# leabouffaut/DAS4Whales

Measured on AMD Instinct MI355X. Metric: channel-samples/sec through f-k filter + matched-filter, higher is better.
Workload: dtype f32 (matched filter: 2 x f16 split operands on the matrix cores, f32 accumulate); 1 GPU; 20000 channels x 120000 samples float32 per GPU, classic f-k fan mask (fk_filter_design defaults), stages fk+mf, HF+LF fin-call templates; api=public, parallelism=independent channel blocks x1

## Files before the change

das4whales_amd/csrc/mm_common.h:

```cpp
#pragma once
#include "fft_radix.h"

namespace d4w {

constexpr float kMmLoScale = 2048.f, kMmLoInv = 1.0f / 2048.f;

#ifdef D4W_EMU
typedef uint16_t mm_half;
struct alignas(16) mm_h8 { uint16_t v[8]; };
struct mm_f4 { float v[4]; };
__device__ __forceinline__ mm_half mm_to_half(float x) { return hipemu::f32_to_f16(x); }
__device__ __forceinline__ float mm_to_float(mm_half h) { return hipemu::f16_to_f32(h); }
__device__ __forceinline__ mm_f4 mm_zero() { return mm_f4{{0.f, 0.f, 0.f, 0.f}}; }
__device__ __forceinline__ mm_f4 mm_mfma(const mm_h8& a, const mm_h8& b, mm_f4 c) {
    hipemu::mfma_f32_16x16x32_f16(a.v, b.v, c.v);
    return c;
}
__device__ __forceinline__ float mm_get(const mm_f4& c, int r) { return c.v[r]; }
__device__ __forceinline__ void mm_set(mm_h8& a, int j, mm_half h) { a.v[j] = h; }
__device__ __forceinline__ int mm_uniform(int v) { return v; }
__device__ __forceinline__ void mm_sched_fence() {}
__device__ __forceinline__ void mm_store4(float* p, float a, float b, float c, float d) { p[0] = a; p[1] = b; p[2] = c; p[3] = d; }
__device__ __forceinline__ void mm_store1(float* p, float v) { *p = v; }
__device__ __forceinline__ float4 mm_load4_stream(const float4* p) { return *p; }
__device__ __forceinline__ void mm_put4(mm_half* p, const mm_half (&h)[4]) { p[0] = h[0]; p[1] = h[1]; p[2] = h[2]; p[3] = h[3]; }
__device__ __forceinline__ float mm_sqrt(float v) { return sqrtf(v); }
__device__ __forceinline__ void mm_wave_sync() { (void)__shfl_xor(0, 1); }
__device__ __forceinline__ float mm_clamp_half(float v) { return fminf(fmaxf(v, -65504.f), 65504.f); }
static inline int mm_num_cus() { return 2; }
#else
typedef _Float16 mm_half;
typedef _Float16 mm_h8 __attribute__((ext_vector_type(8)));
typedef _Float16 mm_h4 __attribute__((ext_vector_type(4)));
typedef float mm_f4 __attribute__((ext_vector_type(4)));
__device__ __forceinline__ mm_half mm_to_half(float x) { return (_Float16)x; }
__device__ __forceinline__ float mm_to_float(mm_half h) { return (float)h; }
__device__ __forceinline__ mm_f4 mm_zero() { mm_f4 z = {0.f, 0.f, 0.f, 0.f}; return z; }
__device__ __forceinline__ mm_f4 mm_mfma(mm_h8 a, mm_h8 b, mm_f4 c) { return __builtin_amdgcn_mfma_f32_16x16x32_f16(a, b, c, 0, 0, 0); }
__device__ __forceinline__ float mm_get(const mm_f4& c, int r) { return c[r]; }
__device__ __forceinline__ void mm_set(mm_h8& a, int j, mm_half h) { a[j] = h; }
__device__ __forceinline__ int mm_uniform(int v) { return __builtin_amdgcn_readfirstlane(v); }
__device__ __forceinline__ void mm_sched_fence() { __builtin_amdgcn_sched_barrier(0); }
__device__ __forceinline__ void mm_store4(float* p, float a, float b, float c, float d) {
    mm_f4 t = {a, b, c, d};
    __builtin_nontemporal_store(t, reinterpret_cast<mm_f4*>(p));
}
__device__ __forceinline__ void mm_store1(float* p, float v) { __builtin_nontemporal_store(v, p); }
__device__ __forceinline__ float4 mm_load4_stream(const float4* p) {
    const mm_f4 v = __builtin_nontemporal_load(reinterpret_cast<const mm_f4*>(p));
    return make_float4(v.x, v.y, v.z, v.w);
}
__device__ __forceinline__ void mm_put4(mm_half* p, const mm_half (&h)[4]) {
    mm_h4 v = {h[0], h[1], h[2], h[3]};
    *reinterpret_cast<mm_h4*>(p) = v;
}
__device__ __forceinline__ float mm_sqrt(float v) { return __builtin_amdgcn_sqrtf(v); }
// ... 74 lines not shown
```

das4whales_amd/csrc/xcorr_mm.hip:

```cpp
#include <cstdlib>

#include "mm_common.h"

namespace d4w {

#ifndef D4W_MM_CH
#define D4W_MM_CH 4096
#endif
constexpr int kMmCH = D4W_MM_CH;
constexpr int kMmKS = 6;
constexpr int kMmKSLong = 8;
constexpr int kMmKSMax = 16;
constexpr int kMmSection = 32 * kMmKSMax - 16;
constexpr int kMmMaxSupport = 32 * kMmKSLong - 15;
constexpr int kMmMaxSections = 16;
constexpr int kMmThreads = 256;
template <int KSM>
struct MmGeom {
    static constexpr int Halo = 32 * KSM;
    static constexpr int Stage = kMmCH + Halo;
    static constexpr int Q = (Stage + 4 * kMmThreads - 1) / (4 * kMmThreads);
    static constexpr int LastQ = (Stage - (Q - 1) * 4 * kMmThreads) / 4;
    static constexpr int Arr = Stage + 8;
};
__host__ __device__ constexpr int mm_pidx(int h) { return h; }

struct MmArgs {
    const float* x;
    const float* xnext;
    const double* mean;
    const float* maxabs;
    const float* taps;
    float* y0;
    float* y1;
    int nx, ns, ld_next, n_next, ltaps, len0, len1;
    float* rowmax0;
    float* rowmax1;
    int clamp;
// ... 12 lines not shown
    return v;
#else
    auto dpp = [](float x, auto ctrl, auto rmask) {
        return __int_as_float(__builtin_amdgcn_update_dpp(0, __float_as_int(x), decltype(ctrl)::value, decltype(rmask)::value, 0xf, false));
    };
    v += dpp(v, std::integral_constant<int, 0x111>{}, std::integral_constant<int, 0xf>{});
    v += dpp(v, std::integral_constant<int, 0x112>{}, std::integral_constant<int, 0xf>{});
    v += dpp(v, std::integral_constant<int, 0x114>{}, std::integral_constant<int, 0xf>{});
    v += dpp(v, std::integral_constant<int, 0x118>{}, std::integral_constant<int, 0xf>{});
    v += dpp(v, std::integral_constant<int, 0x142>{}, std::integral_constant<int, 0xa>{});
    v += dpp(v, std::integral_constant<int, 0x143>{}, std::integral_constant<int, 0xc>{});
    return v;
#endif
}

template <int KS0, int KS1, int WPS, bool TAIL = false, bool WMAX = false, bool WSPLIT = false>
__global__ __launch_bounds__(kMmThreads, WPS) void xcorr_mm_rows(MmArgs P) {
    static_assert(!(WSPLIT && KS1 > 0), "the wave-split kernel is the one-template code run by two wave pairs");
    constexpr int KSM = KS0 > KS1 ? KS0 : KS1;
    using GEO = MmGeom<KSM>;
    constexpr int kMmHalo = GEO::Halo, kMmStage = GEO::Stage, kMmQ = GEO::Q, kMmLastQ = GEO::LastQ, kMmArr = GEO::Arr;
    constexpr int kSeg = 4 * kMmQ;
    D4W_DYN_LDS(smem_raw);
    mm_half* lds = reinterpret_cast<mm_half*>(smem_raw);
    float* red = reinterpret_cast<float*>(lds + 4 * kMmArr);
    constexpr int kBlk = kMmCH / 4;
    float* pb = red + 8;
    float* wt = pb + 2 * kBlk;
    const int tid = (int)threadIdx.x;
    const int lane = tid & 63, wv = mm_uniform(tid >> 6);
    const int n16 = lane & 15, g = lane >> 4;
    const int ns = P.ns;
    const int tsel = WSPLIT ? (wv >> 1) : 0;

    const int nchunk = (ns + kMmCH - 1) / kMmCH;
    const long long total = (long long)P.nx * nchunk;
    const int nparts = min(8, (int)gridDim.x);
    const int xcd = (int)blockIdx.x % nparts, wq = (int)blockIdx.x / nparts, nq = ((int)gridDim.x - xcd + nparts - 1) / nparts;
    const long long lo_c = total * xcd / nparts, hi_c = total * (xcd + 1) / nparts;
    mm_h8 a0h[KS0], a0l[KS0];
    mm_h8 a1h[KS1 ? KS1 : 1], a1l[KS1 ? KS1 : 1];
    float osc0 = 1.f, osc1 = 1.f;
#ifdef D4W_MM_V_TAIL_DEALT
    constexpr bool kRows = false;
#else
    constexpr bool kRows = TAIL;
#endif
    auto next_chunk = [&](long long c) -> long long {
        if constexpr (kRows) {
            const long long r = c / nchunk;
            return (c - r * nchunk + 1 < nchunk) ? c + 1 : (r + (long long)gridDim.x) * nchunk;
        } else {
            return c + nq;
        }
    };
    const long long end_c = kRows ? total : hi_c;
    long long c_n = kRows ? (long long)blockIdx.x * nchunk : lo_c + wq;
    {
        float* tl = reinterpret_cast<float*>(smem_raw);
        constexpr int TLP = 16 + kMmHalo;
        for (int i = tid; i < 2 * TLP; i += kMmThreads) {
            const int t = i / TLP, u = i - t * TLP - 15;
            const int L = t ? P.len1 : P.len0;
            float tv = (u >= 0 && u < L && (t == 0 || KS1 > 0 || WSPLIT)) ? P.taps[(size_t)t * P.ltaps + u] : 0.f;
            if constexpr (TAIL) {
                if (u < L && (t == 0 || KS1 > 0 || WSPLIT)) tv += t ? P.tail1 : P.tail0;
            }
            tl[i] = tv;
        }
        __syncthreads();
        auto build = [&](const float* tp, int L, auto& ah, auto& al, auto ks, float& osc) {
            constexpr int KS = decltype(ks)::value;
// ... 14 lines not shown
                    mm_set(ah[kk], j, hi);
                    mm_set(al[kk], j, lo);
                });
            });
        };
        build(tl + (WSPLIT ? tsel * TLP : 0), WSPLIT && tsel ? P.len1 : P.len0, a0h, a0l, std::integral_constant<int, KS0>{}, osc0);
        if constexpr (KS1 > 0) build(tl + TLP, P.len1, a1h, a1l, std::integral_constant<int, KS1>{}, osc1);
        __syncthreads();
    }

    float4 pre[kMmQ];
    Mean2 mu_n{0.f, 0.f};
    float g_n = 1.f;
    bool heavy_n = false;
    bool tail_n = false;
    int row_n = 0, c0_n = 0;

    auto issue = [&](long long c) {
        row_n = (int)(c / nchunk);
        c0_n = (int)(c - (long long)row_n * nchunk) * kMmCH;
        mu_n = mean2_load(P.mean, row_n);
        g_n = 1.f;
        const int s0 = c0_n + P.shift;
        tail_n = s0 + kMmStage > ns;
        if (P.maxabs) {
            const float a = P.maxabs[row_n];
            g_n = (a > 0.f) ? 1.0f / a : 0.f;
            heavy_n = fabsf(mu_n.hi) > 0.9921875f * a;
        }
        const float* xr = P.x + (size_t)row_n * ns;
        const bool al = (reinterpret_cast<uintptr_t>(xr + s0) & 15) == 0;
        if (al && s0 + kMmStage <= ns) {
            const float4* p = reinterpret_cast<const float4*>(xr + s0) + tid;
            static_for<kMmQ>([&](auto qq) {
                constexpr int q = decltype(qq)::value;
                if (q < kMmQ - 1 || tid < kMmLastQ) pre[q] = mm_load4_stream(p + q * kMmThreads);
            });
        } else {
            if (al && (ns & 3) == 0) {
                static_for<kMmQ>([&](auto qq) {
                    constexpr int q = decltype(qq)::value;
                    if (q < kMmQ - 1 || tid < kMmLastQ) {
                        const int i = s0 + 4 * (tid + q * kMmThreads);
                        const float4 v = *reinterpret_cast<const float4*>(xr + min(i, ns - 4));
                        pre[q] = (i < ns) ? v : make_float4(mu_n.hi, mu_n.hi, mu_n.hi, mu_n.hi);
// ... 16 lines not shown
                    constexpr int q = decltype(qq)::value;
                    if (q < kMmQ - 1 || tid < kMmLastQ) {
                        const int d = s0 + 4 * (tid + q * kMmThreads) - ns;
                        const float b0 = xn[min(max(d, 0), n_next - 1)], b1 = xn[min(max(d + 1, 0), n_next - 1)];
                        const float b2 = xn[min(max(d + 2, 0), n_next - 1)], b3 = xn[min(max(d + 3, 0), n_next - 1)];
                        if (d >= 0 && d < n_next) pre[q].x = b0;
                        if (d + 1 >= 0 && d + 1 < n_next) pre[q].y = b1;
                        if (d + 2 >= 0 && d + 2 < n_next) pre[q].z = b2;
                        if (d + 3 >= 0 && d + 3 < n_next) pre[q].w = b3;
                    }
                });
            }
        }
    };

    if (c_n < end_c) issue(c_n);
    int buf = 0;
    constexpr bool want_max = WMAX;
    float pst_hi = 0.f, pst_lo = 0.f;
    for (long long c = c_n; c < end_c;) {
        const int row = row_n, c0 = c0_n;
        const Mean2 mu = mu_n;
        const bool tail = tail_n;
        const int n_valid = ns + ((P.xnext && P.n_next > 0) ? P.n_next : 0) - c0 - P.shift;
        float gsc = g_n, osx = 1.f;
        const float gout = g_n;
        const bool own_scale = !P.maxabs || heavy_n;
        mm_half* bh = lds + (size_t)buf * 2 * kMmArr;
        mm_half* bl = bh + kMmArr;
        const long long c_next = next_chunk(c);
        const int cin = c0 / kMmCH;
        if (TAIL && cin == 0) { pst_hi = 0.f; pst_lo = 0.f; }
        const float pst = pst_hi;
        if (own_scale) {
            float m = 0.f;
            static_for<kMmQ>([&](auto qq) {
                constexpr int q = decltype(qq)::value;
                if (q < kMmQ - 1 || tid < kMmLastQ) {
                    const float4 v = pre[q];
                    const int at = 4 * (tid + q * kMmThreads);
                    float d0 = demean(v.x, mu), d1 = demean(v.y, mu), d2 = demean(v.z, mu), d3 = demean(v.w, mu);
                    if (tail) {
                        if (at >= n_valid) d0 = 0.f;
                        if (at + 1 >= n_valid) d1 = 0.f;
                        if (at + 2 >= n_valid) d2 = 0.f;
                        if (at + 3 >= n_valid) d3 = 0.f;
                    }
                    m = fmaxf(fmaxf(m, fmaxf(fabsf(d0), fabsf(d1))), fmaxf(fabsf(d2), fabsf(d3)));
                }
            });
            for (int o = 32; o > 0; o >>= 1) m = fmaxf(m, __shfl_xor(m, o));
            if (lane == 0) red[wv + 4 * buf] = m;
            lds_barrier();
            m = fmaxf(fmaxf(red[4 * buf], red[4 * buf + 1]), fmaxf(red[4 * buf + 2], red[4 * buf + 3]));
            mm_pow2_scale(m, osx, gsc);
        }
        const float mlg = -mu.lo * gsc;
        static_for<kMmQ>([&](auto qq) {
            constexpr int q = decltype(qq)::value;
            float s[4] = {0.f, 0.f, 0.f, 0.f};
            const bool mine = q < kMmQ - 1 || tid < kMmLastQ;
            const int at = mm_pidx(4 * (tid + q * kMmThreads));
            if (mine) {
                const float4 v = pre[q];
#ifdef D4W_MM_V_FLOATMEAN
                s[0] = (v.x - mu.hi) * gsc; s[1] = (v.y - mu.hi) * gsc; s[2] = (v.z - mu.hi) * gsc; s[3] = (v.w - mu.hi) * gsc;
#else
                s[0] = fmaf(v.x - mu.hi, gsc, mlg); s[1] = fmaf(v.y - mu.hi, gsc, mlg); s[2] = fmaf(v.z - mu.hi, gsc, mlg); s[3] = fmaf(v.w - mu.hi, gsc, mlg);
#endif
                if (P.clamp && !own_scale) static_for<4>([&](auto ee) { constexpr int e = decltype(ee)::value; s[e] = mm_clamp_half(s[e]); });
                if (tail) {
                    const int a0 = 4 * (tid + q * kMmThreads);
                    static_for<4>([&](auto ee) { constexpr int e = decltype(ee)::value; if (a0 + e >= n_valid) s[e] = 0.f; });
                }
#ifdef D4W_MM_V_OLDSPLIT
                mm_half h[4], l[4];
                static_for<4>([&](auto ee) { constexpr int e = decltype(ee)::value; mm_split(s[e], h[e], l[e]); });
                mm_put4(bh + at, h);
                mm_put4(bl + at, l);
#else
                mm_split_put4(s, bh + at, bl + at);
#endif
            }
#ifdef D4W_MM_V_TAIL_NOSCAN
            if constexpr (false) {
#else
            if constexpr (TAIL && q < kMmCH / (4 * kMmThreads)) {
#endif
                const float t4 = (s[0] + s[1]) + (s[2] + s[3]);
                const float inc = mm_wave_scan(t4);
                pb[buf * kBlk + kMmThreads * q + tid] = inc - t4;
                if (lane == 63) wt[buf * 16 + 4 * q + wv] = inc;
            }
        });
        if (c_next < end_c) issue(c_next);
        lds_barrier();
        float* ya = ((WSPLIT && tsel) ? P.y1 : P.y0) + (size_t)row * ns;
        float* yb = KS1 ? P.y1 + (size_t)row * ns : nullptr;
        const bool valign = ((reinterpret_cast<uintptr_t>(ya + c0) & 15) == 0) && (!KS1 || (reinterpret_cast<uintptr_t>(yb + c0) & 15) == 0);
        const float oxs = (own_scale && P.maxabs) ? osx * gout : osx;
        const float o0 = osc0 * oxs, o1 = osc1 * oxs;
        float segoff = 0.f;
        constexpr int NTW = kMmCH / 256 / (WSPLIT ? 2 : 4), NST = NTW * KSM, PF = 2;
        auto tile_of = [&](int ti) { return WSPLIT ? (wv & 1) + 2 * ti : wv + 4 * ti; };
        auto frag = [&](const mm_half* arr, int T, int kk) -> mm_h8 {
            const int gr = 32 * T + 2 * n16 + g + 4 * kk;
            return *reinterpret_cast<const mm_h8*>(arr + mm_pidx(8 * gr));
        };
        mm_h8 fh[PF + 1], fl[PF + 1];
        static_for<PF>([&](auto ss) {
            constexpr int s_ = decltype(ss)::value;
            fh[s_] = frag(bh, tile_of(s_ / KSM), s_ % KSM);
            fl[s_] = frag(bl, tile_of(s_ / KSM), s_ % KSM);
        });
        mm_f4 c0h = mm_zero(), c0l = mm_zero(), c1h = mm_zero(), c1l = mm_zero();
        float vmax0 = -INFINITY, vmax1 = -INFINITY;
        float vsum = 0.f;
        static_for<NST>([&](auto ss) {
            constexpr int s_ = decltype(ss)::value, ti = s_ / KSM, kk = s_ % KSM;
            if constexpr (s_ + PF < NST) {
                fh[(s_ + PF) % (PF + 1)] = frag(bh, tile_of((s_ + PF) / KSM), (s_ + PF) % KSM);
                fl[(s_ + PF) % (PF + 1)] = frag(bl, tile_of((s_ + PF) / KSM), (s_ + PF) % KSM);
            }
            mm_sched_fence();
            const mm_h8 xh = fh[s_ % (PF + 1)], xl = fl[s_ % (PF + 1)];
            if constexpr (kk < KS0) {
                c0h = mm_mfma(a0h[kk], xh, c0h);
                c0l = mm_mfma(a0h[kk], xl, c0l);
            }
            if constexpr (kk < KS1) {
                c1h = mm_mfma(a1h[kk], xh, c1h);
                c1l = mm_mfma(a1h[kk], xl, c1l);
            }
            if constexpr (kk < KS0) c0l = mm_mfma(a0l[kk], xh, c0l);
            if constexpr (kk < KS1) c1l = mm_mfma(a1l[kk], xh, c1l);
            mm_sched_fence();
            if constexpr (kk == KSM - 1) {
                const int T = tile_of(ti);
                const int kl = 256 * T + 16 * n16 + 4 * g;
                const int k = c0 + kl;
                if constexpr (ti == 0) {
                if constexpr (TAIL) {
                    const float w = lane < 16 ? wt[buf * 16 + lane] : 0.f;
                    const float inc = mm_wave_scan(w);
                    segoff = inc - w;
        #ifdef D4W_EMU
                    const float own = __shfl(inc, 15);
        #else
                    const float own = __builtin_bit_cast(float, __builtin_amdgcn_readlane(__builtin_bit_cast(int, inc), 15));
        #endif
                    const double pd = ((double)pst_hi + (double)pst_lo) + (double)(own * oxs);
                    const float ph = (float)pd, pl2 = (float)(pd - (double)ph);
        #ifdef D4W_EMU
                    pst_hi = ph; pst_lo = pl2;
        #else
                    pst_hi = __builtin_bit_cast(float, __builtin_amdgcn_readfirstlane(__builtin_bit_cast(int, ph)));
                    pst_lo = __builtin_bit_cast(float, __builtin_amdgcn_readfirstlane(__builtin_bit_cast(int, pl2)));
        #endif
                }
                }
                float r0[4], r1[4];
                float a0 = 0.f, a1 = 0.f;
#ifdef D4W_MM_V_TAIL_NOSCAN
                if constexpr (false) {
#else
                if constexpr (TAIL) {
#endif
#ifdef D4W_EMU
                    const float so = __shfl(segoff, T);
#else
                    const float so = __builtin_bit_cast(float, __builtin_amdgcn_readlane(__builtin_bit_cast(int, segoff), T));
#endif
                    const float pbk = fmaf(so + pb[buf * kBlk + kMmThreads * (T >> 2) + 64 * (T & 3) + 4 * n16], oxs, pst);
                    a0 = ((WSPLIT && tsel) ? P.tail1 : P.tail0) * pbk;
                    a1 = P.tail1 * pbk;
                }
                static_for<4>([&](auto rr) {
                    constexpr int r = decltype(rr)::value;
                    r0[r] = fmaf(fmaf(mm_get(c0l, r), kMmLoInv, mm_get(c0h, r)), o0, a0);
                    if constexpr (KS1 > 0) r1[r] = fmaf(fmaf(mm_get(c1l, r), kMmLoInv, mm_get(c1h, r)), o1, a1);
                });
                c0h = mm_zero(); c0l = mm_zero(); c1h = mm_zero(); c1l = mm_zero();
                if (valign && k + 3 < ns) {
                    if (KS1 == 0 && P.accumulate) {
                        const float4 o = mm_load4_stream(reinterpret_cast<const float4*>(ya + k));
                        r0[0] += o.x; r0[1] += o.y; r0[2] += o.z; r0[3] += o.w;
                    }
                    mm_store4(ya + k, r0[0], r0[1], r0[2], r0[3]);
                    if constexpr (KS1 > 0) mm_store4(yb + k, r1[0], r1[1], r1[2], r1[3]);
                    if (want_max) {
                        vmax0 = fmaxf(vmax0, fmaxf(fmaxf(r0[0], r0[1]), fmaxf(r0[2], r0[3])));
#ifndef D4W_MM_V_NONAN
                        vsum += (r0[0] + r0[1]) + (r0[2] + r0[3]);
#endif
                        if constexpr (KS1 > 0) {
                            vmax1 = fmaxf(vmax1, fmaxf(fmaxf(r1[0], r1[1]), fmaxf(r1[2], r1[3])));
#ifndef D4W_MM_V_NONAN
// ... 16 lines not shown
                }
            }
        });
        if (want_max) {
            for (int o = 32; o > 0; o >>= 1) {
                vmax0 = fmaxf(vmax0, __shfl_xor(vmax0, o));
                if constexpr (KS1 > 0) vmax1 = fmaxf(vmax1, __shfl_xor(vmax1, o));
            }
            const bool bad = __any(vsum != vsum);
            if (lane == 0) {
                mm_atomic_fmax(((WSPLIT && tsel) ? P.rowmax1 : P.rowmax0) + row, bad ? __uint_as_float(0x7FC00000u) : vmax0);
                if constexpr (KS1 > 0) mm_atomic_fmax(P.rowmax1 + row, bad ? __uint_as_float(0x7FC00000u) : vmax1);
            }
        }
        buf ^= 1;
        c = c_next;
    }
}

}

using namespace d4w;

extern "C" {

int d4w_xcorr_mm_max_support(void) { return kMmSection * kMmMaxSections; }

#define D4W_MM_LAUNCH(KS0, KS1, WPS, TAIL, grid, lds, stream, Q)                                                              \
    do {                                                                                                                      \
        if ((Q).rowmax0) D4W_LAUNCH((xcorr_mm_rows<KS0, KS1, WPS, TAIL, true>), dim3(grid), dim3(kMmThreads), lds, stream, Q);  \
        else D4W_LAUNCH((xcorr_mm_rows<KS0, KS1, WPS, TAIL, false>), dim3(grid), dim3(kMmThreads), lds, stream, Q);             \
    } while (0)

static int mm_one_template(MmArgs P, const float* taps, int len, float* y, float* rowmax, int grid, void* stream) {
    auto lds_of = [](int arr) { return (size_t)4 * arr * sizeof(mm_half) + 8 * sizeof(float); };
    const int nsec = (len <= 32 * kMmKSMax - 15) ? 1 : ceil_div(len, kMmSection);
    const int per = (nsec == 1) ? len : 16 * ceil_div(ceil_div(len, nsec), 16);
    for (int j = 0; j < nsec; ++j) {
        const int first = j * per;
        MmArgs Q = P;
        Q.taps = taps + first;
        Q.len0 = Q.len1 = std::min(per, len - first);
        Q.y0 = y;
        Q.y1 = nullptr;
        Q.shift = first;
        Q.accumulate = j > 0;
        Q.rowmax0 = (j == nsec - 1) ? rowmax : nullptr;
        Q.rowmax1 = nullptr;
        const int ks = ceil_div(Q.len0 + 15, 32);
        if (ks <= kMmKS)
            D4W_MM_LAUNCH(kMmKS, 0, 3, false, grid, lds_of(MmGeom<kMmKS>::Arr), stream, Q);
        else if (ks <= kMmKSLong)
            D4W_MM_LAUNCH(kMmKSLong, 0, 2, false, grid, lds_of(MmGeom<kMmKSLong>::Arr), stream, Q);
        else if (ks <= 12)
            D4W_MM_LAUNCH(12, 0, 2, false, grid, lds_of(MmGeom<12>::Arr), stream, Q);
        else
            D4W_MM_LAUNCH(kMmKSMax, 0, 2, false, grid, lds_of(MmGeom<kMmKSMax>::Arr), stream, Q);
    }
    return D4W_OK;
}

int d4w_xcorr_mm_f32(const float* x, int nx, int ns, const float* xnext, int ld_next, int n_next, const double* mean,
                     const float* maxabs, const float* taps, int ntpl, int ltaps, int len0, int len1, float* y0, float* y1,
                     void* stream) {
    return d4w_xcorr_mm_rowmax_f32(x, nx, ns, xnext, ld_next, n_next, mean, maxabs, taps, ntpl, ltaps, len0, len1, y0, y1, nullptr,
                                   nullptr, stream);
}

int d4w_xcorr_mm_rowmax_f32(const float* x, int nx, int ns, const float* xnext, int ld_next, int n_next, const double* mean,
                            const float* maxabs, const float* taps, int ntpl, int ltaps, int len0, int len1, float* y0, float* y1,
                            float* rowmax0, float* rowmax1, void* stream) {
    return d4w_xcorr_mm_tail_f32(x, nx, ns, xnext, ld_next, n_next, mean, maxabs, taps, ntpl, ltaps, len0, len1, 0.0, 0.0, y0, y1,
// ... 18 lines not shown
        if (std::max(len0, len1) > d4w_xcorr_mm_tail_max_support())
            return fail(D4W_EINVAL, "with a tail the supports (%d, %d) must be <= %d", len0, len1, d4w_xcorr_mm_tail_max_support());
    }
    MmArgs P;
    P.x = x; P.xnext = xnext; P.mean = mean; P.maxabs = maxabs; P.taps = taps; P.y0 = y0; P.y1 = y1;
    P.nx = nx; P.ns = ns; P.ld_next = ld_next; P.n_next = xnext ? n_next : 0; P.ltaps = ltaps; P.len0 = len0; P.len1 = len1;
    P.shift = 0; P.accumulate = 0;
    static const int env_clamp = [] { const char* v = getenv("D4W_MM_CLAMP"); return v ? atoi(v) : 0; }();
    P.clamp = (xnext != nullptr && n_next > 0) || env_clamp;
    P.rowmax0 = rowmax0; P.rowmax1 = (ntpl == 2) ? rowmax1 : nullptr;
    P.tail0 = (float)tail0; P.tail1 = (float)tail1;
    if (rowmax0) {
        D4W_HIP(hipMemsetD32Async((hipDeviceptr_t)rowmax0, (int)0xFF800000u, (size_t)nx, (hipStream_t)stream));
        if (ntpl == 2) D4W_HIP(hipMemsetD32Async((hipDeviceptr_t)rowmax1, (int)0xFF800000u, (size_t)nx, (hipStream_t)stream));
    }
    const int nchunk = ceil_div(ns, kMmCH);
    const long long total = (long long)nx * nchunk;
    static const int env_wgs = [] { const char* v = getenv("D4W_MM_WGS"); const int n = v ? atoi(v) : 0; return n < 0 ? 0 : (n > 8 ? 8 : n); }();
    const int ks0 = ceil_div(len0 + 15, 32), ks1 = ceil_div(len1 + 15, 32);
    const bool fused = ntpl == 2 && std::max(ks0, ks1) <= kMmKS;
    const int per_cu = env_wgs ? env_wgs : ((ntpl == 1 && ks0 <= kMmKS) ? 3 : 2);
    const int ncu = mm_num_cus();
    const int grid = (int)std::min<long long>(total, (long long)ncu * per_cu);
    auto lds_of = [](int arr, bool tl) {
        return (size_t)4 * arr * sizeof(mm_half) + 8 * sizeof(float) + (tl ? ((size_t)2 * (kMmCH / 4) + 2 * 16) * sizeof(float) : 0);
    };
    static const int fused_form = [] { const char* v = getenv("D4W_MM_FUSED"); return v ? atoi(v) : 2; }();
    const int per_cu_ws = env_wgs ? env_wgs : 3;
#define D4W_MM_LAUNCH_WS(TAIL, grid, lds, Q)                                                                                            \
    do {                                                                                                                                \
        if ((Q).rowmax0) D4W_LAUNCH((xcorr_mm_rows<kMmKS, 0, 3, TAIL, true, true>), dim3(grid), dim3(kMmThreads), lds, stream, Q);       \
        else D4W_LAUNCH((xcorr_mm_rows<kMmKS, 0, 3, TAIL, false, true>), dim3(grid), dim3(kMmThreads), lds, stream, Q);                  \
    } while (0)
    if (tails) {
        const int grid_t = (int)std::min<long long>((long long)nx, (long long)ncu * per_cu);
        if (fused && fused_form != 2) {
            D4W_MM_LAUNCH_WS(true, (int)std::min<long long>((long long)nx, (long long)ncu * per_cu_ws), lds_of(MmGeom<kMmKS>::Arr, true), P);
            return D4W_OK;
        }
        if (fused) {
            const size_t lds = lds_of(MmGeom<kMmKS>::Arr, true);
            if (ks0 <= 5)
                D4W_MM_LAUNCH(5, kMmKS, 2, true, grid_t, lds, stream, P);
            else
                D4W_MM_LAUNCH(kMmKS, kMmKS, 2, true, grid_t, lds, stream, P);
            return D4W_OK;
        }
        for (int t = 0; t < ntpl; ++t) {
            MmArgs Q = P;
            Q.taps = taps + (size_t)t * ltaps;
            Q.len0 = Q.len1 = t ? len1 : len0;
            Q.tail0 = t ? (float)tail1 : (float)tail0;
            Q.tail1 = 0.f;
            Q.y0 = t ? y1 : y0;
            Q.y1 = nullptr;
            Q.rowmax0 = t ? rowmax1 : rowmax0;
            Q.rowmax1 = nullptr;
            const int ks = ceil_div(Q.len0 + 15, 32);
            if (ks <= kMmKS) {
                if (Q.rowmax0)
                    D4W_LAUNCH((xcorr_mm_rows<kMmKS, 0, 2, true, true>), dim3(grid_t), dim3(kMmThreads), lds_of(MmGeom<kMmKS>::Arr, true), stream, Q);
                else
                    D4W_LAUNCH((xcorr_mm_rows<kMmKS, 0, 3, true, false>), dim3(grid_t), dim3(kMmThreads), lds_of(MmGeom<kMmKS>::Arr, true), stream, Q);
            }
            else if (ks <= kMmKSLong)
                D4W_MM_LAUNCH(kMmKSLong, 0, 2, true, grid_t, lds_of(MmGeom<kMmKSLong>::Arr, true), stream, Q);
            else if (ks <= 12)
                D4W_MM_LAUNCH(12, 0, 2, true, grid_t, lds_of(MmGeom<12>::Arr, true), stream, Q);
            else
                D4W_MM_LAUNCH(kMmKSMax, 0, 2, true, grid_t, lds_of(MmGeom<kMmKSMax>::Arr, true), stream, Q);
        }
        return D4W_OK;
    }
    if (!fused) {
        int rc = mm_one_template(P, taps, len0, y0, rowmax0, grid, stream);
        if (rc == D4W_OK && ntpl == 2) rc = mm_one_template(P, taps + ltaps, len1, y1, rowmax1, grid, stream);
        return rc;
    }
    const size_t lds = lds_of(MmGeom<kMmKS>::Arr, false);
    if (fused_form != 2) {
        D4W_MM_LAUNCH_WS(false, (int)std::min<long long>(total, (long long)ncu * per_cu_ws), lds, P);
        return D4W_OK;
    }
    if (ks0 <= 5)
        D4W_MM_LAUNCH(5, kMmKS, 2, false, grid, lds, stream, P);
    else
        D4W_MM_LAUNCH(kMmKS, kMmKS, 2, false, grid, lds, stream, P);
    return D4W_OK;
}

}
```

Baseline: 117.3 billion channel-samples/s.

## Process paired 8192-sample chunks as two halo groups in fused matched filter

The fused two-template matched-filter kernel now handles 8192-sample chunks, split internally into two 4096-sample groups. Each group has its own halo and its own power-of-two scale, so per-block overhead (mean and maxabs loads, barriers, issue logic) is amortized over twice the samples. Chunk iteration switches from a 64-bit divide per chunk to incremental row, chunk and offset counters, and the per-row mean and scale load is skipped for later chunks in row mode. The cost is a larger LDS footprint, which may need the dynamic shared memory attribute and may reduce occupancy, plus extra halo conversion work and more register pressure from the per-group arrays.

```diff
diff --git a/das4whales_amd/csrc/mm_common.h b/das4whales_amd/csrc/mm_common.h
--- a/das4whales_amd/csrc/mm_common.h
+++ b/das4whales_amd/csrc/mm_common.h
@@ -19,6 +19,7 @@
 __device__ __forceinline__ float mm_get(const mm_f4& c, int r) { return c.v[r]; }
 __device__ __forceinline__ void mm_set(mm_h8& a, int j, mm_half h) { a.v[j] = h; }
 __device__ __forceinline__ int mm_uniform(int v) { return v; }
+__device__ __forceinline__ float mm_uniform(float v) { return v; }
 __device__ __forceinline__ void mm_sched_fence() {}
 __device__ __forceinline__ void mm_store4(float* p, float a, float b, float c, float d) { p[0] = a; p[1] = b; p[2] = c; p[3] = d; }
 __device__ __forceinline__ void mm_store1(float* p, float v) { *p = v; }
@@ -40,6 +41,7 @@
 __device__ __forceinline__ float mm_get(const mm_f4& c, int r) { return c[r]; }
 __device__ __forceinline__ void mm_set(mm_h8& a, int j, mm_half h) { a[j] = h; }
 __device__ __forceinline__ int mm_uniform(int v) { return __builtin_amdgcn_readfirstlane(v); }
+__device__ __forceinline__ float mm_uniform(float v) { return __builtin_bit_cast(float, __builtin_amdgcn_readfirstlane(__builtin_bit_cast(int, v))); }
 __device__ __forceinline__ void mm_sched_fence() { __builtin_amdgcn_sched_barrier(0); }
 __device__ __forceinline__ void mm_store4(float* p, float a, float b, float c, float d) {
     mm_f4 t = {a, b, c, d};
diff --git a/das4whales_amd/csrc/xcorr_mm.hip b/das4whales_amd/csrc/xcorr_mm.hip
--- a/das4whales_amd/csrc/xcorr_mm.hip
+++ b/das4whales_amd/csrc/xcorr_mm.hip
@@ -8,6 +8,8 @@
 #define D4W_MM_CH 4096
 #endif
 constexpr int kMmCH = D4W_MM_CH;
+constexpr int kMmCHPair = 8192;
+constexpr int kMmGroup = 4096;
 constexpr int kMmKS = 6;
 constexpr int kMmKSLong = 8;
 constexpr int kMmKSMax = 16;
@@ -15,13 +17,23 @@
 constexpr int kMmMaxSupport = 32 * kMmKSLong - 15;
 constexpr int kMmMaxSections = 16;
 constexpr int kMmThreads = 256;
-template <int KSM>
+template <int KSM, int CH = kMmCH>
 struct MmGeom {
+    static constexpr int G = CH > kMmGroup ? CH / kMmGroup : 1;
+    static constexpr int GL = CH / G;
     static constexpr int Halo = 32 * KSM;
-    static constexpr int Stage = kMmCH + Halo;
+    static constexpr int Stage = CH + Halo;
     static constexpr int Q = (Stage + 4 * kMmThreads - 1) / (4 * kMmThreads);
     static constexpr int LastQ = (Stage - (Q - 1) * 4 * kMmThreads) / 4;
-    static constexpr int Arr = Stage + 8;
+    static constexpr int GStage = GL + Halo;
+    static constexpr int Arr = G * GStage + 8;
+    static constexpr int QG = GL / (4 * kMmThreads);
+    static constexpr int Blk = CH / 4;
+    static constexpr int Pb = G == 1 ? Blk : Blk / 4;
+    static constexpr size_t lds_bytes(bool tail) {
+        return (size_t)4 * Arr * sizeof(mm_half) + 8 * G * sizeof(float) + (tail ? ((size_t)2 * Pb + 2 * 16 * G) * sizeof(float) : 0);
+    }
+    static_assert(CH % (4 * kMmThreads) == 0 && GL % (4 * kMmThreads) == 0 && Halo <= 4 * kMmThreads, "a group is whole loads; its halo lies in one");
 };
 __host__ __device__ constexpr int mm_pidx(int h) { return h; }
 
@@ -64,30 +76,24 @@
 #endif
 }
 
-template <int KS0, int KS1, int WPS, bool TAIL = false, bool WMAX = false, bool WSPLIT = false>
+template <int KS0, int KS1, int WPS, bool TAIL = false, bool WMAX = false, bool WSPLIT = false, int CH = kMmCH>
 __global__ __launch_bounds__(kMmThreads, WPS) void xcorr_mm_rows(MmArgs P) {
     static_assert(!(WSPLIT && KS1 > 0), "the wave-split kernel is the one-template code run by two wave pairs");
     constexpr int KSM = KS0 > KS1 ? KS0 : KS1;
-    using GEO = MmGeom<KSM>;
+    using GEO = MmGeom<KSM, CH>;
     constexpr int kMmHalo = GEO::Halo, kMmStage = GEO::Stage, kMmQ = GEO::Q, kMmLastQ = GEO::LastQ, kMmArr = GEO::Arr;
-    constexpr int kSeg = 4 * kMmQ;
+    constexpr int G = GEO::G, GL = GEO::GL, QG = GEO::QG, kPb = GEO::Pb;
     D4W_DYN_LDS(smem_raw);
     mm_half* lds = reinterpret_cast<mm_half*>(smem_raw);
     float* red = reinterpret_cast<float*>(lds + 4 * kMmArr);
-    constexpr int kBlk = kMmCH / 4;
-    float* pb = red + 8;
-    float* wt = pb + 2 * kBlk;
+    float* pb = red + 8 * G;
+    float* wt = pb + 2 * kPb;
     const int tid = (int)threadIdx.x;
     const int lane = tid & 63, wv = mm_uniform(tid >> 6);
     const int n16 = lane & 15, g = lane >> 4;
     const int ns = P.ns;
     const int tsel = WSPLIT ? (wv >> 1) : 0;
 
-    const int nchunk = (ns + kMmCH - 1) / kMmCH;
-    const long long total = (long long)P.nx * nchunk;
-    const int nparts = min(8, (int)gridDim.x);
-    const int xcd = (int)blockIdx.x % nparts, wq = (int)blockIdx.x / nparts, nq = ((int)gridDim.x - xcd + nparts - 1) / nparts;
-    const long long lo_c = total * xcd / nparts, hi_c = total * (xcd + 1) / nparts;
     mm_h8 a0h[KS0], a0l[KS0];
     mm_h8 a1h[KS1 ? KS1 : 1], a1l[KS1 ? KS1 : 1];
     float osc0 = 1.f, osc1 = 1.f;
@@ -96,16 +102,39 @@
 #else
     constexpr bool kRows = TAIL;
 #endif
-    auto next_chunk = [&](long long c) -> long long {
+    const int nchunk = (ns + CH - 1) / CH;
+    int row_n = 0, cin_n = 0;
+    size_t roff_n = 0;
+    bool more_n = false;
+    int left_n = 0, d_row = 0, d_cin = 0;
+    if constexpr (kRows) {
+        row_n = (int)blockIdx.x;
+        more_n = row_n < P.nx;
+    } else {
+        const long long total = (long long)P.nx * nchunk;
+        const int nparts = min(8, (int)gridDim.x);
+        const int xcd = (int)blockIdx.x % nparts, wq = (int)blockIdx.x / nparts, nq = ((int)gridDim.x - xcd + nparts - 1) / nparts;
+        const long long lo_c = total * xcd / nparts, hi_c = total * (xcd + 1) / nparts;
+        const long long c_first = lo_c + wq;
+        left_n = c_first < hi_c ? (int)((hi_c - c_first + nq - 1) / nq) : 0;
+        row_n = (int)(c_first / nchunk);
+        cin_n = (int)(c_first - (long long)row_n * nchunk);
+        d_row = nq / nchunk;
+        d_cin = nq - d_row * nchunk;
+        more_n = left_n > 0;
+    }
+    roff_n = (size_t)row_n * ns;
+    const size_t d_off = (size_t)(kRows ? (int)gridDim.x : d_row) * ns;
+    auto advance = [&]() {
         if constexpr (kRows) {
-            const long long r = c / nchunk;
-            return (c - r * nchunk + 1 < nchunk) ? c + 1 : (r + (long long)gridDim.x) * nchunk;
+            if (++cin_n == nchunk) { cin_n = 0; row_n += (int)gridDim.x; roff_n += d_off; }
+            more_n = row_n < P.nx;
         } else {
-            return c + nq;
+            cin_n += d_cin; row_n += d_row; roff_n += d_off;
+            if (cin_n >= nchunk) { cin_n -= nchunk; ++row_n; roff_n += (size_t)ns; }
+            more_n = --left_n > 0;
         }
     };
-    const long long end_c = kRows ? total : hi_c;
-    long long c_n = kRows ? (long long)blockIdx.x * nchunk : lo_c + wq;
     {
         float* tl = reinterpret_cast<float*>(smem_raw);
         constexpr int TLP = 16 + kMmHalo;
@@ -150,21 +179,22 @@
     float g_n = 1.f;
     bool heavy_n = false;
     bool tail_n = false;
-    int row_n = 0, c0_n = 0;
-
-    auto issue = [&](long long c) {
-        row_n = (int)(c / nchunk);
-        c0_n = (int)(c - (long long)row_n * nchunk) * kMmCH;
-        mu_n = mean2_load(P.mean, row_n);
-        g_n = 1.f;
+    int c0_n = 0;
+
+    auto issue = [&]() {
+        c0_n = cin_n * CH;
+        if (!kRows || cin_n == 0) {
+            mu_n = mean2_load(P.mean, row_n);
+            g_n = 1.f;
+            if (P.maxabs) {
+                const float a = P.maxabs[row_n];
+                g_n = (a > 0.f) ? 1.0f / a : 0.f;
+                heavy_n = fabsf(mu_n.hi) > 0.9921875f * a;
+            }
+        }
         const int s0 = c0_n + P.shift;
         tail_n = s0 + kMmStage > ns;
-        if (P.maxabs) {
-            const float a = P.maxabs[row_n];
-            g_n = (a > 0.f) ? 1.0f / a : 0.f;
-            heavy_n = fabsf(mu_n.hi) > 0.9921875f * a;
-        }
-        const float* xr = P.x + (size_t)row_n * ns;
+        const float* xr = P.x + roff_n;
         const bool al = (reinterpret_cast<uintptr_t>(xr + s0) & 15) == 0;
         if (al && s0 + kMmStage <= ns) {
             const float4* p = reinterpret_cast<const float4*>(xr + s0) + tid;
@@ -211,28 +241,29 @@
         }
     };
 
-    if (c_n < end_c) issue(c_n);
+    if (more_n) issue();
     int buf = 0;
     constexpr bool want_max = WMAX;
     float pst_hi = 0.f, pst_lo = 0.f;
-    for (long long c = c_n; c < end_c;) {
-        const int row = row_n, c0 = c0_n;
+    for (bool more = more_n; more; more = more_n) {
+        const int row = row_n, c0 = c0_n, cin = cin_n;
+        const size_t roff = roff_n;
         const Mean2 mu = mu_n;
         const bool tail = tail_n;
         const int n_valid = ns + ((P.xnext && P.n_next > 0) ? P.n_next : 0) - c0 - P.shift;
-        float gsc = g_n, osx = 1.f;
         const float gout = g_n;
         const bool own_scale = !P.maxabs || heavy_n;
+        float gsc[G], osx[G];
+        static_for<G>([&](auto gg) { gsc[decltype(gg)::value] = g_n; osx[decltype(gg)::value] = 1.f; });
         mm_half* bh = lds + (size_t)buf * 2 * kMmArr;
         mm_half* bl = bh + kMmArr;
-        const long long c_next = next_chunk(c);
-        const int cin = c0 / kMmCH;
+        advance();
         if (TAIL && cin == 0) { pst_hi = 0.f; pst_lo = 0.f; }
-        const float pst = pst_hi;
         if (own_scale) {
-            float m = 0.f;
+            float m[G];
+            static_for<G>([&](auto gg) { m[decltype(gg)::value] = 0.f; });
             static_for<kMmQ>([&](auto qq) {
-                constexpr int q = decltype(qq)::value;
+                constexpr int q = decltype(qq)::value, gq = q / QG < G ? q / QG : G - 1;
                 if (q < kMmQ - 1 || tid < kMmLastQ) {
                     const float4 v = pre[q];
                     const int at = 4 * (tid + q * kMmThreads);
@@ -243,72 +274,107 @@
                         if (at + 2 >= n_valid) d2 = 0.f;
                         if (at + 3 >= n_valid) d3 = 0.f;
                     }
-                    m = fmaxf(fmaxf(m, fmaxf(fabsf(d0), fabsf(d1))), fmaxf(fabsf(d2), fabsf(d3)));
+                    m[gq] = fmaxf(fmaxf(m[gq], fmaxf(fabsf(d0), fabsf(d1))), fmaxf(fabsf(d2), fabsf(d3)));
+                    if constexpr (q >= QG && q < G * QG && q % QG == 0) {
+                        if (tid < kMmHalo / 4) m[gq - 1] = fmaxf(fmaxf(m[gq - 1], fmaxf(fabsf(d0), fabsf(d1))), fmaxf(fabsf(d2), fabsf(d3)));
+                    }
                 }
             });
-            for (int o = 32; o > 0; o >>= 1) m = fmaxf(m, __shfl_xor(m, o));
-            if (lane == 0) red[wv + 4 * buf] = m;
+            static_for<G>([&](auto gg) {
+                constexpr int gi = decltype(gg)::value;
+                for (int o = 32; o > 0; o >>= 1) m[gi] = fmaxf(m[gi], __shfl_xor(m[gi], o));
+                if (lane == 0) red[wv + 4 * (gi + G * buf)] = m[gi];
+            });
             lds_barrier();
-            m = fmaxf(fmaxf(red[4 * buf], red[4 * buf + 1]), fmaxf(red[4 * buf + 2], red[4 * buf + 3]));
-            mm_pow2_scale(m, osx, gsc);
-        }
-        const float mlg = -mu.lo * gsc;
+            static_for<G>([&](auto gg) {
+                constexpr int gi = decltype(gg)::value;
+                const float* r4 = red + 4 * (gi + G * buf);
+                float up, down;
+                mm_pow2_scale(fmaxf(fmaxf(r4[0], r4[1]), fmaxf(r4[2], r4[3])), up, down);
+                osx[gi] = mm_uniform(up);
+                gsc[gi] = mm_uniform(down);
+            });
+        }
+        auto scaled = [&](const float4 v, int at, auto gg, float (&s)[4]) {
+            constexpr int gi = decltype(gg)::value;
+            const float mlg = -mu.lo * gsc[gi];
+#ifdef D4W_MM_V_FLOATMEAN
+            s[0] = (v.x - mu.hi) * gsc[gi]; s[1] = (v.y - mu.hi) * gsc[gi]; s[2] = (v.z - mu.hi) * gsc[gi]; s[3] = (v.w - mu.hi) * gsc[gi];
+#else
+            s[0] = fmaf(v.x - mu.hi, gsc[gi], mlg); s[1] = fmaf(v.y - mu.hi, gsc[gi], mlg); s[2] = fmaf(v.z - mu.hi, gsc[gi], mlg); s[3] = fmaf(v.w - mu.hi, gsc[gi], mlg);
+#endif
+            if (P.clamp && !own_scale) static_for<4>([&](auto ee) { constexpr int e = decltype(ee)::value; s[e] = mm_clamp_half(s[e]); });
+            if (tail) {
+                static_for<4>([&](auto ee) { constexpr int e = decltype(ee)::value; if (at + e >= n_valid) s[e] = 0.f; });
+            }
+        };
         static_for<kMmQ>([&](auto qq) {
-            constexpr int q = decltype(qq)::value;
+            constexpr int q = decltype(qq)::value, gq = q / QG < G ? q / QG : G - 1;
             float s[4] = {0.f, 0.f, 0.f, 0.f};
             const bool mine = q < kMmQ - 1 || tid < kMmLastQ;
-            const int at = mm_pidx(4 * (tid + q * kMmThreads));
+            const int at = 4 * (tid + q * kMmThreads);
+#ifdef D4W_MM_V_NOCONV
+            if (mine && pre[q].x == 1.2345e30f) {
+#else
             if (mine) {
-                const float4 v = pre[q];
-#ifdef D4W_MM_V_FLOATMEAN
-                s[0] = (v.x - mu.hi) * gsc; s[1] = (v.y - mu.hi) * gsc; s[2] = (v.z - mu.hi) * gsc; s[3] = (v.w - mu.hi) * gsc;
-#else
-                s[0] = fmaf(v.x - mu.hi, gsc, mlg); s[1] = fmaf(v.y - mu.hi, gsc, mlg); s[2] = fmaf(v.z - mu.hi, gsc, mlg); s[3] = fmaf(v.w - mu.hi, gsc, mlg);
-#endif
-                if (P.clamp && !own_scale) static_for<4>([&](auto ee) { constexpr int e = decltype(ee)::value; s[e] = mm_clamp_half(s[e]); });
-                if (tail) {
-                    const int a0 = 4 * (tid + q * kMmThreads);
-                    static_for<4>([&](auto ee) { constexpr int e = decltype(ee)::value; if (a0 + e >= n_valid) s[e] = 0.f; });
-                }
+#endif
+                scaled(pre[q], at, std::integral_constant<int, gq>{}, s);
 #ifdef D4W_MM_V_OLDSPLIT
                 mm_half h[4], l[4];
                 static_for<4>([&](auto ee) { constexpr int e = decltype(ee)::value; mm_split(s[e], h[e], l[e]); });
-                mm_put4(bh + at, h);
-                mm_put4(bl + at, l);
-#else
-                mm_split_put4(s, bh + at, bl + at);
-#endif
+                mm_put4(bh + mm_pidx(at + gq * kMmHalo), h);
+                mm_put4(bl + mm_pidx(at + gq * kMmHalo), l);
+#else
+                mm_split_put4(s, bh + mm_pidx(at + gq * kMmHalo), bl + mm_pidx(at + gq * kMmHalo));
+#endif
+                if constexpr (q >= QG && q < G * QG && q % QG == 0) {
+                    if (tid < kMmHalo / 4) {
+                        float h4[4];
+                        scaled(pre[q], at, std::integral_constant<int, gq - 1>{}, h4);
+                        mm_split_put4(h4, bh + mm_pidx(at + (gq - 1) * kMmHalo), bl + mm_pidx(at + (gq - 1) * kMmHalo));
+                    }
+                }
             }
 #ifdef D4W_MM_V_TAIL_NOSCAN
             if constexpr (false) {
 #else
-            if constexpr (TAIL && q < kMmCH / (4 * kMmThreads)) {
+            if constexpr (TAIL && q < G * QG) {
 #endif
                 const float t4 = (s[0] + s[1]) + (s[2] + s[3]);
                 const float inc = mm_wave_scan(t4);
-                pb[buf * kBlk + kMmThreads * q + tid] = inc - t4;
-                if (lane == 63) wt[buf * 16 + 4 * q + wv] = inc;
+                if constexpr (G == 1) pb[buf * kPb + kMmThreads * q + tid] = inc - t4;
+                else if ((lane & 3) == 0) pb[buf * kPb + (kMmThreads / 4) * q + (tid >> 2)] = inc - t4;
+                if (lane == 63) wt[buf * 16 * G + 4 * q + wv] = inc;
             }
         });
-        if (c_next < end_c) issue(c_next);
+        if (more_n) issue();
         lds_barrier();
-        float* ya = ((WSPLIT && tsel) ? P.y1 : P.y0) + (size_t)row * ns;
-        float* yb = KS1 ? P.y1 + (size_t)row * ns : nullptr;
+        float* ya = ((WSPLIT && tsel) ? P.y1 : P.y0) + roff;
+        float* yb = KS1 ? P.y1 + roff : nullptr;
         const bool valign = ((reinterpret_cast<uintptr_t>(ya + c0) & 15) == 0) && (!KS1 || (reinterpret_cast<uintptr_t>(yb + c0) & 15) == 0);
-        const float oxs = (own_scale && P.maxabs) ? osx * gout : osx;
-        const float o0 = osc0 * oxs, o1 = osc1 * oxs;
-        float segoff = 0.f;
-        constexpr int NTW = kMmCH / 256 / (WSPLIT ? 2 : 4), NST = NTW * KSM, PF = 2;
+        float oxs[G], o0[G], o1[G];
+        static_for<G>([&](auto gg) {
+            constexpr int gi = decltype(gg)::value;
+            oxs[gi] = (own_scale && P.maxabs) ? osx[gi] * gout : osx[gi];
+            o0[gi] = osc0 * oxs[gi];
+            o1[gi] = osc1 * oxs[gi];
+        });
+        float segoff[G], pstg[G];
+        static_for<G>([&](auto gg) { segoff[decltype(gg)::value] = 0.f; pstg[decltype(gg)::value] = 0.f; });
+        constexpr int TPW = WSPLIT ? 2 : 4;
+        constexpr int NTW = CH / 256 / TPW, NST = NTW * KSM, PF = 2;
+        constexpr int TG = GL / 256;
         auto tile_of = [&](int ti) { return WSPLIT ? (wv & 1) + 2 * ti : wv + 4 * ti; };
-        auto frag = [&](const mm_half* arr, int T, int kk) -> mm_h8 {
+        auto frag = [&](const mm_half* arr, int ti, int kk) -> mm_h8 {
+            const int T = tile_of(ti);
             const int gr = 32 * T + 2 * n16 + g + 4 * kk;
-            return *reinterpret_cast<const mm_h8*>(arr + mm_pidx(8 * gr));
+            return *reinterpret_cast<const mm_h8*>(arr + mm_pidx(8 * gr + (TPW * ti / TG) * kMmHalo));
         };
         mm_h8 fh[PF + 1], fl[PF + 1];
         static_for<PF>([&](auto ss) {
             constexpr int s_ = decltype(ss)::value;
-            fh[s_] = frag(bh, tile_of(s_ / KSM), s_ % KSM);
-            fl[s_] = frag(bl, tile_of(s_ / KSM), s_ % KSM);
+            fh[s_] = frag(bh, s_ / KSM, s_ % KSM);
+            fl[s_] = frag(bl, s_ / KSM, s_ % KSM);
         });
         mm_f4 c0h = mm_zero(), c0l = mm_zero(), c1h = mm_zero(), c1l = mm_zero();
         float vmax0 = -INFINITY, vmax1 = -INFINITY;
@@ -316,11 +382,12 @@
         static_for<NST>([&](auto ss) {
             constexpr int s_ = decltype(ss)::value, ti = s_ / KSM, kk = s_ % KSM;
             if constexpr (s_ + PF < NST) {
-                fh[(s_ + PF) % (PF + 1)] = frag(bh, tile_of((s_ + PF) / KSM), (s_ + PF) % KSM);
-                fl[(s_ + PF) % (PF + 1)] = frag(bl, tile_of((s_ + PF) / KSM), (s_ + PF) % KSM);
+                fh[(s_ + PF) % (PF + 1)] = frag(bh, (s_ + PF) / KSM, (s_ + PF) % KSM);
+                fl[(s_ + PF) % (PF + 1)] = frag(bl, (s_ + PF) / KSM, (s_ + PF) % KSM);
             }
             mm_sched_fence();
             const mm_h8 xh = fh[s_ % (PF + 1)], xl = fl[s_ % (PF + 1)];
+#ifndef D4W_MM_V_NOMFMA
             if constexpr (kk < KS0) {
                 c0h = mm_mfma(a0h[kk], xh, c0h);
                 c0l = mm_mfma(a0h[kk], xl, c0l);
@@ -331,30 +398,38 @@
             }
             if constexpr (kk < KS0) c0l = mm_mfma(a0l[kk], xh, c0l);
             if constexpr (kk < KS1) c1l = mm_mfma(a1l[kk], xh, c1l);
+#else
+            c0h[0] += (float)xh[0]; c0l[0] += (float)xl[0];
+#endif
             mm_sched_fence();
             if constexpr (kk == KSM - 1) {
+                constexpr int tg = TPW * ti / TG;
                 const int T = tile_of(ti);
                 const int kl = 256 * T + 16 * n16 + 4 * g;
                 const int k = c0 + kl;
                 if constexpr (ti == 0) {
-                if constexpr (TAIL) {
-                    const float w = lane < 16 ? wt[buf * 16 + lane] : 0.f;
-                    const float inc = mm_wave_scan(w);
-                    segoff = inc - w;
-        #ifdef D4W_EMU
-                    const float own = __shfl(inc, 15);
-        #else
-                    const float own = __builtin_bit_cast(float, __builtin_amdgcn_readlane(__builtin_bit_cast(int, inc), 15));
-        #endif
-                    const double pd = ((double)pst_hi + (double)pst_lo) + (double)(own * oxs);
-                    const float ph = (float)pd, pl2 = (float)(pd - (double)ph);
-        #ifdef D4W_EMU
-                    pst_hi = ph; pst_lo = pl2;
-        #else
-                    pst_hi = __builtin_bit_cast(float, __builtin_amdgcn_readfirstlane(__builtin_bit_cast(int, ph)));
-                    pst_lo = __builtin_bit_cast(float, __builtin_amdgcn_readfirstlane(__builtin_bit_cast(int, pl2)));
-        #endif
-                }
+                    if constexpr (TAIL) {
+                        static_for<G>([&](auto gg) {
+                            constexpr int gi = decltype(gg)::value;
+                            const float w = lane < 16 ? wt[buf * 16 * G + 16 * gi + lane] : 0.f;
+                            const float inc = mm_wave_scan(w);
+                            segoff[gi] = inc - w;
+                            pstg[gi] = pst_hi;
+#ifdef D4W_EMU
+                            const float own = __shfl(inc, 15);
+#else
+                            const float own = __builtin_bit_cast(float, __builtin_amdgcn_readlane(__builtin_bit_cast(int, inc), 15));
+#endif
+                            const double pd = ((double)pst_hi + (double)pst_lo) + (double)(own * oxs[gi]);
+                            const float ph = (float)pd, pl2 = (float)(pd - (double)ph);
+#ifdef D4W_EMU
+                            pst_hi = ph; pst_lo = pl2;
+#else
+                            pst_hi = __builtin_bit_cast(float, __builtin_amdgcn_readfirstlane(__builtin_bit_cast(int, ph)));
+                            pst_lo = __builtin_bit_cast(float, __builtin_amdgcn_readfirstlane(__builtin_bit_cast(int, pl2)));
+#endif
+                        });
+                    }
                 }
                 float r0[4], r1[4];
                 float a0 = 0.f, a1 = 0.f;
@@ -364,20 +439,25 @@
                 if constexpr (TAIL) {
 #endif
 #ifdef D4W_EMU
-                    const float so = __shfl(segoff, T);
-#else
-                    const float so = __builtin_bit_cast(float, __builtin_amdgcn_readlane(__builtin_bit_cast(int, segoff), T));
-#endif
-                    const float pbk = fmaf(so + pb[buf * kBlk + kMmThreads * (T >> 2) + 64 * (T & 3) + 4 * n16], oxs, pst);
+                    const float so = __shfl(segoff[tg], T - tg * TG);
+#else
+                    const float so = __builtin_bit_cast(float, __builtin_amdgcn_readlane(__builtin_bit_cast(int, segoff[tg]), T - tg * TG));
+#endif
+                    const int pi = G == 1 ? kMmThreads * (T >> 2) + 64 * (T & 3) + 4 * n16 : (kMmThreads / 4) * (T >> 2) + 16 * (T & 3) + n16;
+                    const float pbk = fmaf(so + pb[buf * kPb + pi], oxs[tg], pstg[tg]);
                     a0 = ((WSPLIT && tsel) ? P.tail1 : P.tail0) * pbk;
                     a1 = P.tail1 * pbk;
                 }
                 static_for<4>([&](auto rr) {
                     constexpr int r = decltype(rr)::value;
-                    r0[r] = fmaf(fmaf(mm_get(c0l, r), kMmLoInv, mm_get(c0h, r)), o0, a0);
-                    if constexpr (KS1 > 0) r1[r] = fmaf(fmaf(mm_get(c1l, r), kMmLoInv, mm_get(c1h, r)), o1, a1);
+                    r0[r] = fmaf(fmaf(mm_get(c0l, r), kMmLoInv, mm_get(c0h, r)), o0[tg], a0);
+                    if constexpr (KS1 > 0) r1[r] = fmaf(fmaf(mm_get(c1l, r), kMmLoInv, mm_get(c1h, r)), o1[tg], a1);
                 });
                 c0h = mm_zero(); c0l = mm_zero(); c1h = mm_zero(); c1l = mm_zero();
+#ifdef D4W_MM_V_NOSTORE
+                if (r0[0] != 1.2345e30f) { }
+                else
+#endif
                 if (valign && k + 3 < ns) {
                     if (KS1 == 0 && P.accumulate) {
                         const float4 o = mm_load4_stream(reinterpret_cast<const float4*>(ya + k));
@@ -424,7 +504,6 @@
             }
         }
         buf ^= 1;
-        c = c_next;
     }
 }
 
@@ -436,14 +515,16 @@
 
 int d4w_xcorr_mm_max_support(void) { return kMmSection * kMmMaxSections; }
 
-#define D4W_MM_LAUNCH(KS0, KS1, WPS, TAIL, grid, lds, stream, Q)                                                              \
+#define D4W_MM_LAUNCH(KS0, KS1, WPS, TAIL, grid, lds, stream, Q) D4W_MM_LAUNCH_CH(KS0, KS1, WPS, TAIL, kMmCH, grid, lds, stream, Q)
+#define D4W_MM_LAUNCH_CH(KS0, KS1, WPS, TAIL, CH, grid, lds, stream, Q)                                                       \
     do {                                                                                                                      \
-        if ((Q).rowmax0) D4W_LAUNCH((xcorr_mm_rows<KS0, KS1, WPS, TAIL, true>), dim3(grid), dim3(kMmThreads), lds, stream, Q);  \
-        else D4W_LAUNCH((xcorr_mm_rows<KS0, KS1, WPS, TAIL, false>), dim3(grid), dim3(kMmThreads), lds, stream, Q);             \
+        void (*kern_)(MmArgs) = (Q).rowmax0 ? xcorr_mm_rows<KS0, KS1, WPS, TAIL, true, false, CH>                              \
+                                            : xcorr_mm_rows<KS0, KS1, WPS, TAIL, false, false, CH>;                            \
+        if ((lds) > 64 * 1024) D4W_HIP(hipFuncSetAttribute((const void*)kern_, hipFuncAttributeMaxDynamicSharedMemorySize, (int)(lds))); \
+        D4W_LAUNCH(kern_, dim3(grid), dim3(kMmThreads), lds, stream, Q);                                                       \
     } while (0)
 
 static int mm_one_template(MmArgs P, const float* taps, int len, float* y, float* rowmax, int grid, void* stream) {
-    auto lds_of = [](int arr) { return (size_t)4 * arr * sizeof(mm_half) + 8 * sizeof(float); };
     const int nsec = (len <= 32 * kMmKSMax - 15) ? 1 : ceil_div(len, kMmSection);
     const int per = (nsec == 1) ? len : 16 * ceil_div(ceil_div(len, nsec), 16);
     for (int j = 0; j < nsec; ++j) {
@@ -459,13 +540,13 @@
         Q.rowmax1 = nullptr;
         const int ks = ceil_div(Q.len0 + 15, 32);
         if (ks <= kMmKS)
-            D4W_MM_LAUNCH(kMmKS, 0, 3, false, grid, lds_of(MmGeom<kMmKS>::Arr), stream, Q);
+            D4W_MM_LAUNCH(kMmKS, 0, 3, false, grid, MmGeom<kMmKS>::lds_bytes(false), stream, Q);
         else if (ks <= kMmKSLong)
-            D4W_MM_LAUNCH(kMmKSLong, 0, 2, false, grid, lds_of(MmGeom<kMmKSLong>::Arr), stream, Q);
+            D4W_MM_LAUNCH(kMmKSLong, 0, 2, false, grid, MmGeom<kMmKSLong>::lds_bytes(false), stream, Q);
         else if (ks <= 12)
-            D4W_MM_LAUNCH(12, 0, 2, false, grid, lds_of(MmGeom<12>::Arr), stream, Q);
+            D4W_MM_LAUNCH(12, 0, 2, false, grid, MmGeom<12>::lds_bytes(false), stream, Q);
         else
-            D4W_MM_LAUNCH(kMmKSMax, 0, 2, false, grid, lds_of(MmGeom<kMmKSMax>::Arr), stream, Q);
+            D4W_MM_LAUNCH(kMmKSMax, 0, 2, false, grid, MmGeom<kMmKSMax>::lds_bytes(false), stream, Q);
     }
     return D4W_OK;
 }
@@ -514,18 +595,15 @@
         D4W_HIP(hipMemsetD32Async((hipDeviceptr_t)rowmax0, (int)0xFF800000u, (size_t)nx, (hipStream_t)stream));
         if (ntpl == 2) D4W_HIP(hipMemsetD32Async((hipDeviceptr_t)rowmax1, (int)0xFF800000u, (size_t)nx, (hipStream_t)stream));
     }
-    const int nchunk = ceil_div(ns, kMmCH);
-    const long long total = (long long)nx * nchunk;
     static const int env_wgs = [] { const char* v = getenv("D4W_MM_WGS"); const int n = v ? atoi(v) : 0; return n < 0 ? 0 : (n > 8 ? 8 : n); }();
     const int ks0 = ceil_div(len0 + 15, 32), ks1 = ceil_div(len1 + 15, 32);
     const bool fused = ntpl == 2 && std::max(ks0, ks1) <= kMmKS;
+    static const int fused_form = [] { const char* v = getenv("D4W_MM_FUSED"); return v ? atoi(v) : 2; }();
+    const int nchunk = ceil_div(ns, (fused && fused_form == 2) ? kMmCHPair : kMmCH);
+    const long long total = (long long)nx * nchunk;
     const int per_cu = env_wgs ? env_wgs : ((ntpl == 1 && ks0 <= kMmKS) ? 3 : 2);
     const int ncu = mm_num_cus();
     const int grid = (int)std::min<long long>(total, (long long)ncu * per_cu);
-    auto lds_of = [](int arr, bool tl) {
-        return (size_t)4 * arr * sizeof(mm_half) + 8 * sizeof(float) + (tl ? ((size_t)2 * (kMmCH / 4) + 2 * 16) * sizeof(float) : 0);
-    };
-    static const int fused_form = [] { const char* v = getenv("D4W_MM_FUSED"); return v ? atoi(v) : 2; }();
     const int per_cu_ws = env_wgs ? env_wgs : 3;
 #define D4W_MM_LAUNCH_WS(TAIL, grid, lds, Q)                                                                                            \
     do {                                                                                                                                \
@@ -535,15 +613,15 @@
     if (tails) {
         const int grid_t = (int)std::min<long long>((long long)nx, (long long)ncu * per_cu);
         if (fused && fused_form != 2) {
-            D4W_MM_LAUNCH_WS(true, (int)std::min<long long>((long long)nx, (long long)ncu * per_cu_ws), lds_of(MmGeom<kMmKS>::Arr, true), P);
+            D4W_MM_LAUNCH_WS(true, (int)std::min<long long>((long long)nx, (long long)ncu * per_cu_ws), MmGeom<kMmKS>::lds_bytes(true), P);
             return D4W_OK;
         }
         if (fused) {
-            const size_t lds = lds_of(MmGeom<kMmKS>::Arr, true);
+            const size_t lds = MmGeom<kMmKS, kMmCHPair>::lds_bytes(true);
             if (ks0 <= 5)
-                D4W_MM_LAUNCH(5, kMmKS, 2, true, grid_t, lds, stream, P);
+                D4W_MM_LAUNCH_CH(5, kMmKS, 2, true, kMmCHPair, grid_t, lds, stream, P);
             else
-                D4W_MM_LAUNCH(kMmKS, kMmKS, 2, true, grid_t, lds, stream, P);
+                D4W_MM_LAUNCH_CH(kMmKS, kMmKS, 2, true, kMmCHPair, grid_t, lds, stream, P);
             return D4W_OK;
         }
         for (int t = 0; t < ntpl; ++t) {
@@ -559,16 +637,16 @@
             const int ks = ceil_div(Q.len0 + 15, 32);
             if (ks <= kMmKS) {
                 if (Q.rowmax0)
-                    D4W_LAUNCH((xcorr_mm_rows<kMmKS, 0, 2, true, true>), dim3(grid_t), dim3(kMmThreads), lds_of(MmGeom<kMmKS>::Arr, true), stream, Q);
+                    D4W_LAUNCH((xcorr_mm_rows<kMmKS, 0, 2, true, true>), dim3(grid_t), dim3(kMmThreads), MmGeom<kMmKS>::lds_bytes(true), stream, Q);
                 else
-                    D4W_LAUNCH((xcorr_mm_rows<kMmKS, 0, 3, true, false>), dim3(grid_t), dim3(kMmThreads), lds_of(MmGeom<kMmKS>::Arr, true), stream, Q);
+                    D4W_LAUNCH((xcorr_mm_rows<kMmKS, 0, 3, true, false>), dim3(grid_t), dim3(kMmThreads), MmGeom<kMmKS>::lds_bytes(true), stream, Q);
             }
             else if (ks <= kMmKSLong)
-                D4W_MM_LAUNCH(kMmKSLong, 0, 2, true, grid_t, lds_of(MmGeom<kMmKSLong>::Arr, true), stream, Q);
+                D4W_MM_LAUNCH(kMmKSLong, 0, 2, true, grid_t, MmGeom<kMmKSLong>::lds_bytes(true), stream, Q);
             else if (ks <= 12)
-                D4W_MM_LAUNCH(12, 0, 2, true, grid_t, lds_of(MmGeom<12>::Arr, true), stream, Q);
+                D4W_MM_LAUNCH(12, 0, 2, true, grid_t, MmGeom<12>::lds_bytes(true), stream, Q);
             else
-                D4W_MM_LAUNCH(kMmKSMax, 0, 2, true, grid_t, lds_of(MmGeom<kMmKSMax>::Arr, true), stream, Q);
+                D4W_MM_LAUNCH(kMmKSMax, 0, 2, true, grid_t, MmGeom<kMmKSMax>::lds_bytes(true), stream, Q);
         }
         return D4W_OK;
     }
@@ -577,15 +655,15 @@
         if (rc == D4W_OK && ntpl == 2) rc = mm_one_template(P, taps + ltaps, len1, y1, rowmax1, grid, stream);
         return rc;
     }
-    const size_t lds = lds_of(MmGeom<kMmKS>::Arr, false);
     if (fused_form != 2) {
-        D4W_MM_LAUNCH_WS(false, (int)std::min<long long>(total, (long long)ncu * per_cu_ws), lds, P);
+        D4W_MM_LAUNCH_WS(false, (int)std::min<long long>(total, (long long)ncu * per_cu_ws), MmGeom<kMmKS>::lds_bytes(false), P);
         return D4W_OK;
     }
+    const size_t lds = MmGeom<kMmKS, kMmCHPair>::lds_bytes(false);
     if (ks0 <= 5)
-        D4W_MM_LAUNCH(5, kMmKS, 2, false, grid, lds, stream, P);
+        D4W_MM_LAUNCH_CH(5, kMmKS, 2, false, kMmCHPair, grid, lds, stream, P);
     else
-        D4W_MM_LAUNCH(kMmKS, kMmKS, 2, false, grid, lds, stream, P);
+        D4W_MM_LAUNCH_CH(kMmKS, kMmKS, 2, false, kMmCHPair, grid, lds, stream, P);
     return D4W_OK;
 }
 
```

Measured after the change: 120.2 billion channel-samples/s, median of 6. 2.5% higher.
